# hanzz2007/libxsmm-1

Hardware: AMD Instinct MI355X
Metric: batched SMM fp32 32x32x32 GFLOP/s (whole job) (higher is better)
Workload: dtype f32; 1 GPU; configs[1]: batched dense SMM fp32 M=N=K=32 alpha=1 beta=1, batch=1048576 per GPU, strided addressing, MFMA on; batch_per_gpu=1048576, parallelism=batch-shard x1

## Files before the change

libxsmm-1_amd/csrc/kernels/smm_special.hip:

```cpp
#include "smm_common.cuh"
#include <mutex>

namespace xsmm {
namespace {

typedef float f32x4 __attribute__((ext_vector_type(4)));
typedef float f32x16 __attribute__((ext_vector_type(16)));
typedef double f64x4 __attribute__((ext_vector_type(4)));

__device__ __forceinline__ bool aligned16(const void* p) { return 0 == (reinterpret_cast<uintptr_t>(p) & 15); }

template<bool GLB> struct Space { typedef float* ptr; typedef const float* cptr; typedef f32x4* vptr; typedef const f32x4* cvptr; };
template<> struct Space<true> {
  typedef __attribute__((address_space(1))) float* ptr; typedef const __attribute__((address_space(1))) float* cptr;
  typedef __attribute__((address_space(1))) f32x4* vptr; typedef const __attribute__((address_space(1))) f32x4* cvptr;
};
template<bool NT, bool GLB> __device__ __forceinline__ f32x4 ld4(const float* p, bool al)
{
  const typename Space<GLB>::cptr g = (typename Space<GLB>::cptr)p;
  if (al) return NT ? __builtin_nontemporal_load((typename Space<GLB>::cvptr)g) : *(typename Space<GLB>::cvptr)g;
  return f32x4{ g[0], g[1], g[2], g[3] };
}
template<bool NT, bool GLB> __device__ __forceinline__ void st4(float* p, bool al, f32x4 v)
{
  const typename Space<GLB>::ptr g = (typename Space<GLB>::ptr)p;
  if (al) { if (NT) __builtin_nontemporal_store(v, (typename Space<GLB>::vptr)g); else *(typename Space<GLB>::vptr)g = v; }
  else { g[0] = v[0]; g[1] = v[1]; g[2] = v[2]; g[3] = v[3]; }
}
template<bool NT, bool GLB> __device__ __forceinline__ float ld1(const float* p) { const typename Space<GLB>::cptr g = (typename Space<GLB>::cptr)p; return NT ? __builtin_nontemporal_load(g) : *g; }
template<bool NT, bool GLB> __device__ __forceinline__ void st1(float* p, float v) { const typename Space<GLB>::ptr g = (typename Space<GLB>::ptr)p; if (NT) __builtin_nontemporal_store(v, g); else *g = v; }

template<bool NT, bool GLB> __device__ __forceinline__ void load_mat32(const float* p, int lane, f32x4 (&r)[4])
{
  const bool al = aligned16(p);
#pragma unroll
  for (int j = 0; j < 4; ++j) r[j] = ld4<NT, GLB>(p + 4 * (64 * j + lane), al);
}

template<int KEYSHIFT> __device__ __forceinline__ void park_ab(float* As, float* Bs, int lane, const f32x4 (&ra)[4], const f32x4 (&rb)[4])
{
#pragma unroll
  for (int j = 0; j < 4; ++j) {
    const int c = 64 * j + lane;
    *reinterpret_cast<f32x4*>(As + 4 * c) = ra[j];
    const int n = c >> 3, q = c & 7;
    *reinterpret_cast<f32x4*>(Bs + 4 * (n * 8 + (q ^ ((n >> KEYSHIFT) & 7)))) = rb[j];
  }
}

template<bool BETA0, bool NT, bool GLB>
__global__ __launch_bounds__(256, 4)
void smm32_f32_fma_kernel(DevAddr ad, long long batch)
{
  __shared__ __align__(16) float lds[4][2048];
  const int wave = __builtin_amdgcn_readfirstlane(threadIdx.x >> 6), lane = threadIdx.x & 63;
  const int tx = lane & 7, ty = lane >> 3;
  float* const As = lds[wave];
  float* const Bs = lds[wave] + 1024;
  const long long w = (long long)blockIdx.x * 4 + wave, W = (long long)gridDim.x * 4;
  if (w >= batch) return;

  f32x4 ra[4], rb[4], rc[4];
  load_mat32<NT, GLB>(addr_a<float>(ad, w), lane, ra);
  load_mat32<NT, GLB>(addr_b<float>(ad, w), lane, rb);
  if (!BETA0) {
    const float* const pc = addr_c<float>(ad, w) + 4 * ty * 32 + 4 * tx;
    const bool al = aligned16(pc);
#pragma unroll
    for (int j = 0; j < 4; ++j) rc[j] = ld4<NT, GLB>(pc + j * 32, al);
  }
  for (long long item = w; item < batch; item += W) {
    float* const pc = addr_c<float>(ad, item) + 4 * ty * 32 + 4 * tx;
    park_ab<2>(As, Bs, lane, ra, rb);
    f32x4 acc[4];
#pragma unroll
    for (int j = 0; j < 4; ++j) acc[j] = BETA0 ? f32x4{ 0.f, 0.f, 0.f, 0.f } : rc[j];
    const long long next = item + W;
    if (next < batch) {
      load_mat32<NT, GLB>(addr_a<float>(ad, next), lane, ra);
      load_mat32<NT, GLB>(addr_b<float>(ad, next), lane, rb);
      if (!BETA0) {
        const float* const pn = addr_c<float>(ad, next) + 4 * ty * 32 + 4 * tx;
        const bool al = aligned16(pn);
#pragma unroll
        for (int j = 0; j < 4; ++j) rc[j] = ld4<NT, GLB>(pn + j * 32, al);
      }
    }
    wave_lds_sync();
#pragma unroll 2
    for (int q = 0; q < 8; ++q) {
      f32x4 av[4], bv[4];
#pragma unroll
      for (int kk = 0; kk < 4; ++kk) av[kk] = *reinterpret_cast<const f32x4*>(As + (4 * q + kk) * 32 + 4 * tx);
#pragma unroll
      for (int j = 0; j < 4; ++j) bv[j] = *reinterpret_cast<const f32x4*>(Bs + 4 * ((4 * ty + j) * 8 + (q ^ ty)));
#pragma unroll
      for (int kk = 0; kk < 4; ++kk) {
#pragma unroll
        for (int j = 0; j < 4; ++j) {
#pragma unroll
          for (int i = 0; i < 4; ++i) acc[j][i] = xfma(av[kk][i], bv[j][kk], acc[j][i]);
        }
      }
    }
    const bool al = aligned16(pc);
#pragma unroll
    for (int j = 0; j < 4; ++j) st4<NT, GLB>(pc + j * 32, al, acc[j]);
    wave_lds_sync();
  }
}

template<bool BETA0, bool NT, bool GLB, bool RUNS>
__global__ __launch_bounds__(256, 4)
void smm32_f32_mfma_kernel(DevAddr ad, long long batch, int runlen)
{
  __shared__ __align__(16) float lds[4][2048];
  const int wave = __builtin_amdgcn_readfirstlane(threadIdx.x >> 6), lane = threadIdx.x & 63;
  const int lo = lane & 31, hi = lane >> 5;
  float* const As = lds[wave];
  float* const Bs = lds[wave] + 1024;
  const long long w = (long long)blockIdx.x * 4 + wave, W = (long long)gridDim.x * 4;
  const long long nunits = RUNS ? batch / runlen : batch;
  if (w >= nunits) return;
  const int coff = 4 * hi * 32 + lo;

  f32x4 ra[4], rb[4];
  float rc[16];
  auto load_c = [&](const float* pc) {
#pragma unroll
    for (int r = 0; r < 16; ++r) rc[r] = ld1<NT, GLB>(pc + ((r & 3) + 8 * (r >> 2)) * 32);
  };
  long long unit = w;
  int r0 = 0;
  auto step = [&](long long u, int r, long long& u1, int& r1) { r1 = RUNS ? r + 1 : 0; u1 = u; if (!RUNS || r1 == runlen) { r1 = 0; u1 += W; } };
  float* pc_cur; float* pc_nxt = nullptr;
  {
    const long long first = RUNS ? unit * runlen : unit;
    load_mat32<NT, GLB>(addr_a<float>(ad, first), lane, ra);
    load_mat32<NT, GLB>(addr_b<float>(ad, first), lane, rb);
    pc_cur = addr_c<float>(ad, first);
    if (!BETA0) load_c(pc_cur + coff);
  }
  long long raw_a = 0, raw_b = 0, raw_c = 0;
  if (!RUNS && unit + W < nunits) {
    raw_a = raw_of(ad.a, ad.ia, ad.sa, ad, unit + W); raw_b = raw_of(ad.b, ad.ib, ad.sb, ad, unit + W); raw_c = raw_of(ad.c, ad.ic, ad.sc, ad, unit + W);
  }
  f32x16 acc;
  f32x16 pend; float* pend_pc = nullptr;
  auto store_pend = [&]() {
#pragma unroll
    for (int r = 0; r < 16; ++r) st1<NT, GLB>(pend_pc + ((r & 3) + 8 * (r >> 2)) * 32, pend[r]);
  };
  for (;;) {
    __builtin_amdgcn_s_waitcnt(0x0F70);
    if (nullptr != pend_pc) { store_pend(); pend_pc = nullptr; }
    park_ab<1>(As, Bs, lane, ra, rb);
    if (!RUNS || 0 == r0) {
#pragma unroll
      for (int r = 0; r < 16; ++r) acc[r] = BETA0 ? 0.f : rc[r];
    }
    int r1; long long unit1; step(unit, r0, unit1, r1);
    const bool more = unit1 < nunits;
    if (more) {
      if (RUNS) {
        const long long next = unit1 * runlen + r1;
        load_mat32<NT, GLB>(addr_a<float>(ad, next), lane, ra);
        load_mat32<NT, GLB>(addr_b<float>(ad, next), lane, rb);
        if (0 == r1) { pc_nxt = addr_c<float>(ad, next); if (!BETA0) load_c(pc_nxt + coff); } else pc_nxt = pc_cur;
      }
      else {
        load_mat32<NT, GLB>(cooked<const float>(ad.a, ad, raw_a), lane, ra);
        load_mat32<NT, GLB>(cooked<const float>(ad.b, ad, raw_b), lane, rb);
        pc_nxt = cooked<float>(ad.c, ad, raw_c);
        if (!BETA0) load_c(pc_nxt + coff);
        const long long next2 = unit1 + W;
        if (next2 < nunits) { raw_a = raw_of(ad.a, ad.ia, ad.sa, ad, next2); raw_b = raw_of(ad.b, ad.ib, ad.sb, ad, next2); raw_c = raw_of(ad.c, ad.ic, ad.sc, ad, next2); }
      }
    }
    wave_lds_sync();
    f32x4 bt[8];
#pragma unroll
    for (int t = 0; t < 8; ++t) bt[t] = *reinterpret_cast<const f32x4*>(Bs + 4 * (lo * 8 + (t ^ ((lo >> 1) & 7))));
#pragma unroll
    for (int s = 0; s < 16; ++s) {
      const float av = As[(2 * s + hi) * 32 + lo];
      const float bv = (0 != hi) ? bt[s >> 1][2 * (s & 1) + 1] : bt[s >> 1][2 * (s & 1)];
      acc = __builtin_amdgcn_mfma_f32_32x32x2f32(bv, av, acc, 0, 0, 0);
    }
    if (!RUNS || r0 + 1 == runlen) { pend = acc; pend_pc = pc_cur + coff; }
    wave_lds_sync();
    if (!more) break;
    unit = unit1; r0 = r1; pc_cur = pc_nxt;
  }
  if (nullptr != pend_pc) store_pend();
}

template<bool BETA0>
__global__ __launch_bounds__(256, 4)
void smm64_f32_mfma_kernel(DevAddr ad, long long batch)
{
  __shared__ __align__(16) float As[4096];
  __shared__ __align__(16) float Bs[4096];
  const int t = threadIdx.x, wave = __builtin_amdgcn_readfirstlane(t >> 6), lane = t & 63, lo = lane & 31, hi = lane >> 5;
  const int mq = wave & 1, nq = wave >> 1;
  const int m = 32 * mq + lo, n = 32 * nq + lo;
  const int coff = (32 * nq + 4 * hi) * 64 + m;
  long long item = blockIdx.x;
  if (item >= batch) return;

  f32x4 ra[4], rb[4];
  float rc[16];
  auto load_ab = [&](long long i) {
    const float* const pa = addr_a<float>(ad, i);
    const float* const pb = addr_b<float>(ad, i);
    const bool ala = aligned16(pa), alb = aligned16(pb);
#pragma unroll
    for (int j = 0; j < 4; ++j) {
      ra[j] = ld4<true, false>(pa + 4 * (256 * j + t), ala);
      rb[j] = ld4<true, false>(pb + 4 * (256 * j + t), alb);
    }
  };
  auto load_c = [&](const float* pc) {
#pragma unroll
    for (int r = 0; r < 16; ++r) rc[r] = ld1<true, false>(pc + ((r & 3) + 8 * (r >> 2)) * 64);
  };
  load_ab(item);
  if (!BETA0) load_c(addr_c<float>(ad, item) + coff);
  for (; item < batch; item += gridDim.x) {
    float* const pc = addr_c<float>(ad, item) + coff;
#pragma unroll
    for (int j = 0; j < 4; ++j) {
      const int c = 256 * j + t, row = c >> 4, q = c & 15;
      *reinterpret_cast<f32x4*>(As + row * 64 + ((4 * q) ^ ((row & 1) << 5))) = ra[j];
      *reinterpret_cast<f32x4*>(Bs + row * 64 + 4 * (q ^ (row & 15))) = rb[j];
    }
    f32x16 acc;
#pragma unroll
    for (int r = 0; r < 16; ++r) acc[r] = BETA0 ? 0.f : rc[r];
    const long long next = item + gridDim.x;
    if (next < batch) {
      load_ab(next);
      if (!BETA0) load_c(addr_c<float>(ad, next) + coff);
    }
    __syncthreads();
#pragma unroll
    for (int half = 0; half < 2; ++half) {
      f32x4 bt[8];
#pragma unroll
      for (int u = 0; u < 8; ++u) bt[u] = *reinterpret_cast<const f32x4*>(Bs + n * 64 + 4 * ((8 * half + u) ^ (n & 15)));
#pragma unroll
      for (int s = 0; s < 16; ++s) {
        const float av = As[(32 * half + 2 * s + hi) * 64 + (m ^ (hi << 5))];
        const float bv = (0 != hi) ? bt[s >> 1][2 * (s & 1) + 1] : bt[s >> 1][2 * (s & 1)];
        acc = __builtin_amdgcn_mfma_f32_32x32x2f32(bv, av, acc, 0, 0, 0);
      }
    }
#pragma unroll
    for (int r = 0; r < 16; ++r) st1<true, false>(pc + ((r & 3) + 8 * (r >> 2)) * 64, acc[r]);
    __syncthreads();
  }
}

#include "smm_mfma_wg.inc"

__global__ __launch_bounds__(256)
void stream_abc_kernel(const f32x4* __restrict__ a, const f32x4* __restrict__ b, f32x4* __restrict__ c, long long items)
{
  const int lane = threadIdx.x & 63;
  const long long w = (long long)blockIdx.x * (blockDim.x >> 6) + __builtin_amdgcn_readfirstlane(threadIdx.x >> 6), W = ((long long)gridDim.x * blockDim.x) >> 6;
  if (w >= items) return;
  f32x4 ra[4], rb[4], rc[4];
#pragma unroll
  for (int j = 0; j < 4; ++j) {
    const long long o = w * 256 + 64 * j + lane;
    ra[j] = __builtin_nontemporal_load(a + o); rb[j] = __builtin_nontemporal_load(b + o); rc[j] = __builtin_nontemporal_load(c + o);
  }
  for (long long it = w; it < items; it += W) {
    f32x4 r[4];
#pragma unroll
    for (int j = 0; j < 4; ++j) r[j] = ra[j] + rb[j] + rc[j];
    const long long nx = it + W;
    if (nx < items) {
#pragma unroll
      for (int j = 0; j < 4; ++j) {
        const long long o = nx * 256 + 64 * j + lane;
        ra[j] = __builtin_nontemporal_load(a + o); rb[j] = __builtin_nontemporal_load(b + o); rc[j] = __builtin_nontemporal_load(c + o);
      }
    }
#pragma unroll
    for (int j = 0; j < 4; ++j) __builtin_nontemporal_store(r[j], c + it * 256 + 64 * j + lane);
  }
}

int env_int(const char* name, int fallback)
{
  const char* const v = getenv(name);
  return (nullptr != v && 0 != *v) ? atoi(v) : fallback;
}

bool is_smm32_f32(const SmmBatch& s)
{
  return 4 == s.typesize && 32 == s.m && 32 == s.n && 32 == s.k && 32 == s.lda && 32 == s.ldb && 32 == s.ldc
      && 0 == (s.flags & LIBXSMM_GEMM_FLAG_TRANS_B) && SYNC_NONE == s.sync && 0 == s.general;
}

bool is_smm64(const SmmBatch& s, int typesize)
{
  return typesize == s.typesize && 64 == s.m && 64 == s.n && 64 == s.k && 64 == s.lda && 64 == s.ldb && 64 == s.ldc
      && 0 == (s.flags & LIBXSMM_GEMM_FLAG_TRANS_B) && SYNC_NONE == s.sync && 0 == s.general && 0 != s.use_mfma;
}

long long mfma_wg_units(const SmmBatch& s)
{
  if (SYNC_NONE == s.sync) return s.batch;
  if (SYNC_RUNS == s.sync && 0 < s.uniform_run && 0 == s.batch % s.uniform_run) return s.batch / s.uniform_run;
  return 0;
}
int mfma_wg_runlen(const SmmBatch& s) { return SYNC_NONE == s.sync ? 1 : s.uniform_run; }

template<bool NT, bool GLB>
int launch_smm32(const SmmBatch& s, hipStream_t st, unsigned blocks, const char** name)
{
  const bool beta0 = (0 != (s.flags & LIBXSMM_GEMM_FLAG_BETA_0));
  const DevAddr ad = make_addr(s);
  if (0 == s.use_mfma) {
    *name = "smm_f32_32x32x32_fma";
    if (beta0) hipLaunchKernelGGL((smm32_f32_fma_kernel<true, NT, GLB>), dim3(blocks), dim3(256), 0, st, ad, s.batch);
    else hipLaunchKernelGGL((smm32_f32_fma_kernel<false, NT, GLB>), dim3(blocks), dim3(256), 0, st, ad, s.batch);
  }
  else {
    *name = "smm_f32_32x32x32_mfma";
    if (beta0) hipLaunchKernelGGL((smm32_f32_mfma_kernel<true, NT, GLB, false>), dim3(blocks), dim3(256), 0, st, ad, s.batch, 1);
    else hipLaunchKernelGGL((smm32_f32_mfma_kernel<false, NT, GLB, false>), dim3(blocks), dim3(256), 0, st, ad, s.batch, 1);
  }
  return (int)hipGetLastError();
}

}

int launch_smm_special(const SmmBatch& s, void* stream, const char** name)
{
  hipStream_t st = (hipStream_t)stream;
  if (is_smm32_f32(s)) {
    const int bpc = env_int("XSMM_SMM32_BPC", (ADDR_STRIDED == s.mode || 0 == s.use_mfma) ? 3 : 4), nt = env_int("XSMM_SMM32_NT", 1);
    const int variant = env_int("XSMM_SMM32_VARIANT", 0 != s.use_mfma ? 0 : 1);
    long long blocks = (s.batch + 3) / 4;
    const int grid_env = env_int("XSMM_SMM32_GRID", 0);
    const long long resident = (0 < grid_env) ? grid_env : 256LL * (bpc > 0 ? bpc : 3);
    if (blocks > resident) blocks = resident;
    if (1 == variant) return (0 != nt) ? launch_smm32<true, true>(s, st, (unsigned)blocks, name) : launch_smm32<false, true>(s, st, (unsigned)blocks, name);
    return (0 != nt) ? launch_smm32<true, false>(s, st, (unsigned)blocks, name) : launch_smm32<false, false>(s, st, (unsigned)blocks, name);
  }
  if (4 == s.typesize && 32 == s.m && 32 == s.n && 32 == s.k && 32 == s.lda && 32 == s.ldb && 32 == s.ldc && 0 == (s.flags & LIBXSMM_GEMM_FLAG_TRANS_B)
    && SYNC_RUNS == s.sync && 0 < s.uniform_run && 0 == s.batch % s.uniform_run && 0 == s.general && 0 != s.use_mfma && 0 != env_int("XSMM_SMM32_RUNS", 1))
  {
    const long long units = s.batch / s.uniform_run;
    const int bpc = env_int("XSMM_SMM32_RUNS_BPC", 4);
    long long blocks = (units + 3) / 4;
    const long long resident = 256LL * (bpc > 0 ? bpc : 4);
    if (blocks > resident) blocks = resident;
    if (blocks < 1) return -1;
    const DevAddr ad = make_addr(s);
    *name = "smm_f32_32x32x32_mfma_runs";
    if (0 != (s.flags & LIBXSMM_GEMM_FLAG_BETA_0)) hipLaunchKernelGGL((smm32_f32_mfma_kernel<true, false, true, true>), dim3((unsigned)blocks), dim3(256), 0, st, ad, s.batch, s.uniform_run);
    else hipLaunchKernelGGL((smm32_f32_mfma_kernel<false, false, true, true>), dim3((unsigned)blocks), dim3(256), 0, st, ad, s.batch, s.uniform_run);
    return (int)hipGetLastError();
  }
  if (is_smm64(s, 4) && 0 != env_int("XSMM_SMM64_MFMA", 1) && 0 != env_int("XSMM_SMM64_TIGHT", 1)) {
    const int bpc = env_int("XSMM_SMM64_BPC", 4);
    long long blocks = s.batch;
    const long long resident = 256LL * (bpc > 0 ? bpc : 3);
    if (blocks > resident) blocks = resident;
    if (blocks < 1) return -1;
    const DevAddr ad = make_addr(s);
    *name = "smm_f32_64x64x64_mfma";
    if (0 != (s.flags & LIBXSMM_GEMM_FLAG_BETA_0)) hipLaunchKernelGGL((smm64_f32_mfma_kernel<true>), dim3((unsigned)blocks), dim3(256), 0, st, ad, s.batch);
    else hipLaunchKernelGGL((smm64_f32_mfma_kernel<false>), dim3((unsigned)blocks), dim3(256), 0, st, ad, s.batch);
    return (int)hipGetLastError();
  }
  if (4 == s.typesize && (32 < s.m || 32 < s.n) && s.m <= 64 && s.n <= 64 && 0 < s.k && s.k <= 64 && s.lda >= s.m && s.ldb >= s.k && s.ldc >= s.m
    && 0 == (s.flags & LIBXSMM_GEMM_FLAG_TRANS_B) && mfma_wg_units(s) > 0 && 0 == s.general && 0 != s.use_mfma && 0 != env_int("XSMM_SMM64_MFMA", 1))
  {
    const bool tightc = s.ldc == s.m && 0 == ((s.m * s.n) & 3) && 0 != (s.m & 31) && 0 != env_int("XSMM_SMM64_TIGHTC", 1);
    const int bpc = env_int("XSMM_SMM64_BPC", tightc ? 3 : 4);
    long long blocks = mfma_wg_units(s);
    const long long resident = 256LL * (bpc > 0 ? bpc : 4);
    if (blocks > resident) blocks = resident;
    if (blocks < 1) return -1;
    const DevAddr ad = make_addr(s);
    const int runlen = mfma_wg_runlen(s);
    *name = (1 == runlen) ? "smm_f32_mfma_wg" : "smm_f32_mfma_wg_runs";
    const bool beta0 = 0 != (s.flags & LIBXSMM_GEMM_FLAG_BETA_0);
    const bool tight = s.lda == s.m && s.ldb == s.k && 0 == ((s.m * s.k) & 3) && 0 == ((s.k * s.n) & 3) && 0 != env_int("XSMM_SMM64_WIDE", 1);
#define XSMM_MW(B0, TI, TC) hipLaunchKernelGGL((smm_f32_mfma_wg_kernel<B0, TI, TC>), dim3((unsigned)blocks), dim3(256), 0, st, ad, s.m, s.n, s.k, s.lda, s.ldb, s.ldc, s.batch, runlen)
    if (tightc) { if (tight) { if (beta0) XSMM_MW(true, true, true); else XSMM_MW(false, true, true); } else { if (beta0) XSMM_MW(true, false, true); else XSMM_MW(false, false, true); } }
    else { if (tight) { if (beta0) XSMM_MW(true, true, false); else XSMM_MW(false, true, false); } else { if (beta0) XSMM_MW(true, false, false); else XSMM_MW(false, false, false); } }
#undef XSMM_MW
    return (int)hipGetLastError();
  }
  if (8 == s.typesize && (32 < s.m || 32 < s.n) && s.m <= 64 && s.n <= 64 && 0 < s.k && s.k <= 64 && s.lda >= s.m && s.ldb >= s.k && s.ldc >= s.m
    && 0 == (s.flags & LIBXSMM_GEMM_FLAG_TRANS_B) && mfma_wg_units(s) > 0 && 0 == s.general && 0 != s.use_mfma && 0 != env_int("XSMM_SMM64_MFMA", 1))
  {
    const bool two = s.k > 32 && 0 != env_int("XSMM_SMM64_TWOSTAGE", 1);
    const size_t lds = two ? (size_t)2 * 32 * 64 * sizeof(double) : (size_t)2 * (4 * ((s.k + 3) / 4)) * 64 * sizeof(double);
    int fit = (int)((160u * 1024u) / lds);
    if (fit > 3) fit = 3;
    const int bpc = env_int("XSMM_SMM64_BPC", fit);
    long long blocks = mfma_wg_units(s);
    const long long resident = 256LL * (bpc > 0 ? bpc : fit);
    if (blocks > resident) blocks = resident;
    if (blocks < 1) return -1;
    const DevAddr ad = make_addr(s);
    const int runlen = mfma_wg_runlen(s);
    *name = (1 == runlen) ? "smm_f64_mfma_wg" : "smm_f64_mfma_wg_runs";
    static std::once_flag once;
    std::call_once(once, []() {
      (void)hipFuncSetAttribute(reinterpret_cast<const void*>(&smm_f64_mfma_wg_kernel<true>), hipFuncAttributeMaxDynamicSharedMemorySize, 64 * 1024);
      (void)hipFuncSetAttribute(reinterpret_cast<const void*>(&smm_f64_mfma_wg_kernel<false>), hipFuncAttributeMaxDynamicSharedMemorySize, 64 * 1024);
    });
    if (two) {
      if (0 != (s.flags & LIBXSMM_GEMM_FLAG_BETA_0)) hipLaunchKernelGGL((smm_f64_mfma_wg2_kernel<true>), dim3((unsigned)blocks), dim3(256), lds, st, ad, s.m, s.n, s.k, s.lda, s.ldb, s.ldc, s.batch, runlen);
      else hipLaunchKernelGGL((smm_f64_mfma_wg2_kernel<false>), dim3((unsigned)blocks), dim3(256), lds, st, ad, s.m, s.n, s.k, s.lda, s.ldb, s.ldc, s.batch, runlen);
      return (int)hipGetLastError();
    }
    if (0 != (s.flags & LIBXSMM_GEMM_FLAG_BETA_0)) hipLaunchKernelGGL((smm_f64_mfma_wg_kernel<true>), dim3((unsigned)blocks), dim3(256), lds, st, ad, s.m, s.n, s.k, s.lda, s.ldb, s.ldc, s.batch, runlen);
    else hipLaunchKernelGGL((smm_f64_mfma_wg_kernel<false>), dim3((unsigned)blocks), dim3(256), lds, st, ad, s.m, s.n, s.k, s.lda, s.ldb, s.ldc, s.batch, runlen);
    return (int)hipGetLastError();
  }
  return -1;
}

int launch_stream_abc(const void* a, const void* b, void* c, long long bytes, void* stream)
{
  const long long items = bytes / 4096;
  const int bpc = env_int("XSMM_STREAM_BPC", 3);
  hipLaunchKernelGGL(stream_abc_kernel, dim3(256u * (unsigned)(bpc > 0 ? bpc : 3)), dim3(256), 0, (hipStream_t)stream,
    (const f32x4*)a, (const f32x4*)b, (f32x4*)c, items);
  return (int)hipGetLastError();
}

}
```

Before: 23240 GFLOP/s.

## Add dedicated strided MFMA kernel with grouped prefetch and chunked batch mapping

Adds a specialised kernel for strided, 16-byte-aligned 32x32x32 fp32 batches. It takes raw base pointers and strides, and each wave software-pipelines its items: loads for the next item are split into groups and interleaved with the MFMA steps, and the previous C tile is stored late. A new wave-to-item mapping gives each of 8 block groups a contiguous slice of the batch. It also changes the default grid to one block per CU (256 blocks), which reduces resident waves and leans on the in-wave pipelining to hide latency.

```diff
diff --git a/libxsmm-1_amd/csrc/kernels/smm_special.hip b/libxsmm-1_amd/csrc/kernels/smm_special.hip
--- a/libxsmm-1_amd/csrc/kernels/smm_special.hip
+++ b/libxsmm-1_amd/csrc/kernels/smm_special.hip
@@ -195,6 +195,103 @@
   if (nullptr != pend_pc) store_pend();
 }
 
+__device__ __forceinline__ void wave_walk(int map, long long batch, long long& first, long long& step, long long& end)
+{
+  const int wave = __builtin_amdgcn_readfirstlane(threadIdx.x >> 6);
+  const int nb = (int)gridDim.x, blk = (int)blockIdx.x;
+  step = 4LL * nb; end = batch; first = 4LL * blk + wave;
+  if (0 == map || 0 != (nb & 7)) return;
+  const int g = blk & 7, r = blk >> 3, per = nb >> 3;
+  if (3 == map) {
+    first = batch * g / 8 + 4LL * r + wave; step = 4LL * per; end = batch * (g + 1) / 8;
+    return;
+  }
+  const int p = (1 == map) ? 4 : per;
+  if (0 != per % p) return;
+  first = 4LL * ((long long)((r / p) * 8 + g) * p + r % p) + wave;
+}
+
+template<bool BETA0, int GROUPS, bool CFIRST, bool SMID>
+__global__ __launch_bounds__(256, 4)
+void smm32_f32_mfma_strided_kernel(const float* a0, const float* b0, float* c0, long long sa, long long sb, long long sc, long long batch, int map)
+{
+  static_assert(1 == GROUPS || 2 == GROUPS || 4 == GROUPS || 12 == GROUPS, "12 KiB in equal groups of whole KiB");
+  typedef Space<true>::cptr gcptr; typedef Space<true>::ptr gptr; typedef Space<true>::cvptr gcvptr;
+  __shared__ __align__(16) float lds[4][2048];
+  const int wave = __builtin_amdgcn_readfirstlane(threadIdx.x >> 6), lane = threadIdx.x & 63;
+  const int lo = lane & 31, hi = lane >> 5;
+  float* const As = lds[wave];
+  float* const Bs = lds[wave] + 1024;
+  long long item, step, end;
+  wave_walk(map, batch, item, step, end);
+  if (item >= end) return;
+  const gcptr ga = (gcptr)a0; const gcptr gb = (gcptr)b0; const gptr gc = (gptr)c0;
+  const int coff = 4 * hi * 32 + lo;
+
+  f32x4 ra[4], rb[4];
+  float rc[16];
+  auto load_unit = [&](int u, long long i) {
+    const int cu = CFIRST ? u : u - 8, au = CFIRST ? u - 4 : u;
+    if (0 <= cu && cu < 4) {
+#pragma unroll
+      for (int r = 4 * cu; r < 4 * cu + 4; ++r) rc[r] = __builtin_nontemporal_load(gc + i * sc + coff + ((r & 3) + 8 * (r >> 2)) * 32);
+    }
+    else if (au < 4) ra[au] = __builtin_nontemporal_load((gcvptr)(ga + i * sa) + 64 * au + lane);
+    else rb[au - 4] = __builtin_nontemporal_load((gcvptr)(gb + i * sb) + 64 * (au - 4) + lane);
+  };
+  auto skip_c = [](int u) { return BETA0 && (CFIRST ? u < 4 : u >= 8); };
+#pragma unroll
+  for (int u = 0; u < 12; ++u) if (!skip_c(u)) load_unit(u, item);
+
+  f32x16 pend;
+  long long pend_item = 0;
+  auto store_pend = [&]() {
+#pragma unroll
+    for (int r = 0; r < 16; ++r) __builtin_nontemporal_store(pend[r], gc + pend_item * sc + coff + ((r & 3) + 8 * (r >> 2)) * 32);
+  };
+  auto body = [&](auto loads, auto stores) {
+    constexpr bool LOADS = decltype(loads)::value, STORES = decltype(stores)::value;
+    if (STORES && !SMID) store_pend();
+    __builtin_amdgcn_sched_barrier(0);
+    park_ab<1>(As, Bs, lane, ra, rb);
+    f32x16 acc;
+#pragma unroll
+    for (int r = 0; r < 16; ++r) acc[r] = BETA0 ? 0.f : rc[r];
+    const long long next = item + step;
+    wave_lds_sync();
+    f32x4 bt[8];
+#pragma unroll
+    for (int t = 0; t < 8; ++t) bt[t] = *reinterpret_cast<const f32x4*>(Bs + 4 * (lo * 8 + (t ^ ((lo >> 1) & 7))));
+#pragma unroll
+    for (int g = 0; g < GROUPS; ++g) {
+      if (LOADS) {
+        if (0 < g) __builtin_amdgcn_s_waitcnt(0x0F70);
+#pragma unroll
+        for (int u = g * (12 / GROUPS); u < (g + 1) * (12 / GROUPS); ++u) if (!skip_c(u)) load_unit(u, next);
+        __builtin_amdgcn_sched_barrier(0);
+      }
+      if (STORES && SMID && 0 == g) { store_pend(); __builtin_amdgcn_sched_barrier(0); }
+#pragma unroll
+      for (int s = 16 * g / GROUPS; s < 16 * (g + 1) / GROUPS; ++s) {
+        const float av = As[(2 * s + hi) * 32 + lo];
+        const float bv = (0 != hi) ? bt[s >> 1][2 * (s & 1) + 1] : bt[s >> 1][2 * (s & 1)];
+        acc = __builtin_amdgcn_mfma_f32_32x32x2f32(bv, av, acc, 0, 0, 0);
+      }
+    }
+    pend = acc; pend_item = item;
+    wave_lds_sync();
+    item = next;
+  };
+  typedef std::integral_constant<bool, true> yes; typedef std::integral_constant<bool, false> no;
+  if (item + step < end) {
+    body(yes(), no());
+    while (item + step < end) body(yes(), yes());
+    body(no(), yes());
+  }
+  else body(no(), no());
+  store_pend();
+}
+
 template<bool BETA0>
 __global__ __launch_bounds__(256, 4)
 void smm64_f32_mfma_kernel(DevAddr ad, long long batch)
@@ -329,11 +426,38 @@
     else hipLaunchKernelGGL((smm32_f32_fma_kernel<false, NT, GLB>), dim3(blocks), dim3(256), 0, st, ad, s.batch);
   }
   else {
-    *name = "smm_f32_32x32x32_mfma";
+    *name = "smm_f32_32x32x32_mfma_generic";
     if (beta0) hipLaunchKernelGGL((smm32_f32_mfma_kernel<true, NT, GLB, false>), dim3(blocks), dim3(256), 0, st, ad, s.batch, 1);
     else hipLaunchKernelGGL((smm32_f32_mfma_kernel<false, NT, GLB, false>), dim3(blocks), dim3(256), 0, st, ad, s.batch, 1);
   }
   return (int)hipGetLastError();
+}
+
+bool smm32_strided_ok(const SmmBatch& s)
+{
+  const auto al16 = [](const void* p) { return 0 == (reinterpret_cast<uintptr_t>(p) & 15); };
+  return ADDR_STRIDED == s.mode && 0 != s.use_mfma && al16(s.a) && al16(s.b) && al16(s.c) && 0 == (s.sa & 3) && 0 == (s.sb & 3) && 0 == (s.sc & 3);
+}
+
+template<bool BETA0, int GROUPS>
+void launch_smm32_strided_g(const SmmBatch& s, hipStream_t st, unsigned blocks, int cfirst, int smid, int map)
+{
+#define XSMM_S32(CF, SM) hipLaunchKernelGGL((smm32_f32_mfma_strided_kernel<BETA0, GROUPS, CF, SM>), dim3(blocks), dim3(256), 0, st, \
+  (const float*)s.a, (const float*)s.b, (float*)s.c, s.sa, s.sb, s.sc, s.batch, map)
+  if (0 != cfirst) { if (0 != smid) XSMM_S32(true, true); else XSMM_S32(true, false); }
+  else { if (0 != smid) XSMM_S32(false, true); else XSMM_S32(false, false); }
+#undef XSMM_S32
+}
+
+template<bool BETA0>
+void launch_smm32_strided_b(const SmmBatch& s, hipStream_t st, unsigned blocks, int groups, int cfirst, int smid, int map)
+{
+  switch (groups) {
+    case 1: launch_smm32_strided_g<BETA0, 1>(s, st, blocks, cfirst, smid, map); break;
+    case 2: launch_smm32_strided_g<BETA0, 2>(s, st, blocks, cfirst, smid, map); break;
+    case 4: launch_smm32_strided_g<BETA0, 4>(s, st, blocks, cfirst, smid, map); break;
+    default: launch_smm32_strided_g<BETA0, 12>(s, st, blocks, cfirst, smid, map); break;
+  }
 }
 
 }
@@ -348,6 +472,18 @@
     const int grid_env = env_int("XSMM_SMM32_GRID", 0);
     const long long resident = (0 < grid_env) ? grid_env : 256LL * (bpc > 0 ? bpc : 3);
     if (blocks > resident) blocks = resident;
+    if (smm32_strided_ok(s) && 0 != env_int("XSMM_SMM32_STRIDED", 1)) {
+      const int groups = env_int("XSMM_SMM32_GROUPS", 2), cfirst = env_int("XSMM_SMM32_CFIRST", 1);
+      const int smid = env_int("XSMM_SMM32_SMID", 0), map = env_int("XSMM_SMM32_MAP", 3);
+      if (0 >= env_int("XSMM_SMM32_GRID", 0)) {
+        const long long bl = (s.batch + 3) / 4, res = 256LL * env_int("XSMM_SMM32_BPC", 1);
+        blocks = (bl < res) ? bl : res;
+      }
+      *name = "smm_f32_32x32x32_mfma";
+      if (0 != (s.flags & LIBXSMM_GEMM_FLAG_BETA_0)) launch_smm32_strided_b<true>(s, st, (unsigned)blocks, groups, cfirst, smid, map);
+      else launch_smm32_strided_b<false>(s, st, (unsigned)blocks, groups, cfirst, smid, map);
+      return (int)hipGetLastError();
+    }
     if (1 == variant) return (0 != nt) ? launch_smm32<true, true>(s, st, (unsigned)blocks, name) : launch_smm32<false, true>(s, st, (unsigned)blocks, name);
     return (0 != nt) ? launch_smm32<true, false>(s, st, (unsigned)blocks, name) : launch_smm32<false, false>(s, st, (unsigned)blocks, name);
   }
```

Measured after the change: 23480 GFLOP/s (median of 6 runs). +1.0%, better.
